# Wangshihu12/Voxel-SLAM

Hardware: AMD Instinct MI355X
Metric: local-BA iterations/sec (200k pts, W=10) (higher is better)
Workload: dtype f64

## Files before the change

include/voxelba.h:

```cpp
#ifndef VOXELBA_H
#define VOXELBA_H

#include <stddef.h>
#include <stdint.h>

#ifdef __cplusplus
extern "C" {
#endif

#define VBA_CLUSTER_LEN 10
#define VBA_POSE_LEN 12
#define VBA_STATE_LEN 25
#define VBA_IMU_PRE_LEN 304
#define VBA_DIM 15
#define VBA_MAX_WIN 16

enum vba_status {
  VBA_OK = 0,
  VBA_ERR_NO_DEVICE = 1,
  VBA_ERR_BAD_ARG = 2,
  VBA_ERR_UNSUPPORTED_WINDOW = 3,
  VBA_ERR_TOO_FEW_VOXELS = 4,
  VBA_ERR_OPT_STATE = 5,
  VBA_ERR_HIP = 6,
  VBA_ERR_CAPACITY = 7,
  VBA_ERR_IO = 8,
  VBA_ERR_UNSUPPORTED = 9,
  VBA_ERR_SINGULAR = 10
};

typedef struct vba_ctx vba_ctx;

typedef struct vba_options {
  int win_size;
  double voxel_size;
  int max_layer;
  int max_points;
  double min_eigen_value;
  double plane_eigen_value_thre[4];
  double min_point[4];
  double imu_coef;
  int thread_num;
  int device;
  void *stream;
  size_t max_voxels;
  size_t max_points_per_scan;
  int lm_spec;
  int force_collective;
  int hessian_workgroups;
  int residual_vpl_from;
  int hessian_compact_tiles;
  size_t max_map_nodes;
  size_t max_fix_points;
  int hba_workers;
  int deterministic;
} vba_options;

void vba_default_options(vba_options *opt);
int vba_create(const vba_options *opt, vba_ctx **out);
void vba_destroy(vba_ctx *ctx);
const char *vba_status_string(int status);
const char *vba_last_error(vba_ctx *ctx);
int vba_synchronize(vba_ctx *ctx);


int vba_factor_clear(vba_ctx *ctx);
int vba_factor_push_voxels(vba_ctx *ctx, int n, const double *clusters, const double *fix, const double *coe,
                           const double *eig_val, const double *eig_vec, const double *pcr_add);
int vba_factor_size(vba_ctx *ctx);
int vba_factor_acc_evaluate2(vba_ctx *ctx, const double *poses, int head, int end, double *Hess, double *JacT,
                             double *residual);
int vba_factor_evaluate_only_residual(vba_ctx *ctx, const double *poses, int head, int end, double *residual);
int vba_factor_read_back(vba_ctx *ctx, double *eig_val, double *eig_vec, double *pcr_add);

int vba_factor_occupied_slots(vba_ctx *ctx, long long *slots);
int vba_factor_occupancy_masks(vba_ctx *ctx, unsigned int *masks);


int vba_lidar_ba_damping_iter(vba_ctx *ctx, double *poses, double *hess, double *resis2, int max_iter, int thd_num,
                              int *is_converge);

int vba_li_ba_damping_iter(vba_ctx *ctx, double *states, double *imus, int gravity, int max_iter, double *hess,
                           double *resis2);

// ... 367 lines not shown
```

voxel-slam_amd/capi.py:

```python
from __future__ import annotations

import ctypes as C
import os
import subprocess

import numpy as np

from .abi import KINDS, PROTOTYPES

_PKG = os.path.dirname(os.path.abspath(__file__))
LIB_PATH = os.environ.get("VBA_LIB") or os.path.join(_PKG, "libvoxelba.so")
_dp = C.POINTER(C.c_double)

OK = 0
ERR_NO_DEVICE, ERR_BAD_ARG, ERR_UNSUPPORTED_WINDOW, ERR_TOO_FEW_VOXELS, ERR_OPT_STATE, ERR_HIP, ERR_CAPACITY, ERR_IO, ERR_UNSUPPORTED, ERR_SINGULAR = range(1, 11)

EXPORTS = list(PROTOTYPES)


class Options(C.Structure):
    _fields_ = [
        ("win_size", C.c_int), ("voxel_size", C.c_double), ("max_layer", C.c_int), ("max_points", C.c_int),
        ("min_eigen_value", C.c_double), ("plane_eigen_value_thre", C.c_double * 4), ("min_point", C.c_double * 4),
        ("imu_coef", C.c_double), ("thread_num", C.c_int), ("device", C.c_int), ("stream", C.c_void_p),
        ("max_voxels", C.c_size_t), ("max_points_per_scan", C.c_size_t),
        ("lm_spec", C.c_int), ("force_collective", C.c_int), ("hessian_workgroups", C.c_int), ("residual_vpl_from", C.c_int), ("hessian_compact_tiles", C.c_int),
        ("max_map_nodes", C.c_size_t), ("max_fix_points", C.c_size_t), ("hba_workers", C.c_int),
        ("deterministic", C.c_int),
    ]


class BtcConfig(C.Structure):
    _fields_ = [
        ("skip_near_num", C.c_int), ("candidate_num", C.c_int), ("rough_dis_threshold", C.c_float),
        ("similarity_threshold", C.c_float), ("icp_threshold", C.c_float), ("normal_threshold", C.c_float),
        ("dis_threshold", C.c_float), ("occupy_len", C.c_int),
    ]


class BtcResult(C.Structure):
    _fields_ = [("loop_id", C.c_int), ("score", C.c_double), ("t", C.c_double * 3), ("R", C.c_double * 9)]


class BtcIcpState(C.Structure):
    _fields_ = [("R", C.c_double * 9), ("t", C.c_double * 3), ("paras", C.c_double * 4), ("is_conv", C.c_int), ("done", C.c_int),
                ("iters", C.c_int), ("pad", C.c_int), ("mat", C.c_double * 6), ("eig", C.c_double * 3)]

    @classmethod
    def start(cls, t, R, paras=(0.2, 0.2, 0.5, 3.0), is_conv=0, done=0, iters=0):
        s = cls()
        s.R[:] = [float(x) for x in np.reshape(R, 9)]; s.t[:] = [float(x) for x in np.reshape(t, 3)]
        s.paras[:] = [float(x) for x in paras]
        s.is_conv, s.done, s.iters = int(is_conv), int(done), int(iters)
        return s


class BtcCandidate(C.Structure):
    _fields_ = [("frame", C.c_int), ("votes", C.c_int), ("match_len", C.c_int), ("max_vote_index", C.c_int),
                ("max_vote", C.c_int), ("score", C.c_double)]
# ... 1454 lines not shown
```

voxel-slam_amd/csrc/vba_ctx.hpp:

```cpp
#pragma once
#include "../../include/voxelba.h"
#include "vba_types.hpp"
#include "vba_common.hpp"
#include "vba_mem.hpp"
#include "vba_stores.hpp"
#include "vba_launch.hpp"

#include <hip/hip_runtime.h>
#include <rccl/rccl.h>
#include <array>
#include <cstdlib>
#include <map>
#include <string>
#include <vector>

using namespace vba;

#define VBA_HIPCHK(err, expr)                                                                    \
  do {                                                                                           \
    hipError_t _e = (expr);                                                                      \
    if (_e != hipSuccess) {                                                                      \
      hipchk_err(err) = std::string(#expr) + ": " + hipGetErrorString(_e);                       \
      return VBA_ERR_HIP;                                                                        \
    }                                                                                            \
// ... 19 lines not shown
}
}
namespace vbh { struct OdomEkf; }
struct CtxSat;

struct vba_ctx {
  vba_options opt;
  int device = 0;
  hipStream_t stream = nullptr;
  bool own_stream = false;
  std::string err;

  FactorView fv{};
  DevMem<double> fv_rows[6];
  DevMem<unsigned int> fv_occ;
  DevMem<int> fv_tiles;
  int nvox = 0;
  int nvox_global = 0;
  int cap = 0;
  DevMem<double> d_poses;
  DevMem<double> d_partial;
  DevMem<double> d_out;
  DevMem<double> d_full;
  DevMem<double> d_scal;
  PinMem<double> h_pin;
  DevMem<char> d_stage;

  vba_allreduce_fn allreduce = nullptr;
  void *allreduce_user = nullptr;
  int rank = 0, n_ranks = 1;
  bool force_collective = false;
  int max_blocks_hess = 256;
  int residual_vpl_from = 45000;
  bool use_h3 = false;
  ncclComm_t comm = nullptr;
  bool own_comm = false;
  bool collective_off = false;
  bool collective() const { return !collective_off && (allreduce || comm) && (n_ranks > 1 || force_collective); }

  bool timing = false;
  std::string timing_only;
  int timing_every = 1; unsigned timing_ctr = 0;
  int lm_spec = LM_SPEC;
  std::vector<std::array<double, 450>> covinv_cache; size_t covinv_next = 0;
  std::map<std::string, std::vector<TimedSpan>> spans;

  DevMem<LmDev> d_lm;
  PinMem<LmDev> h_lm;
  struct { bool pending = false; int dbg = 0; double x[VBA_MAX_WIN_DEV * 12]; } lm_init;
  DevMem<double> d_raw;
  struct { bool active = false; int thd_num = 2; bool have_hess = false; bool pending_update = false; int k4_nb = 0; } lm;
  DevMem<double> d_k4part;
  std::vector<double> trace;

  DevMem<LiDev> d_li;
  DevMem<double> d_imu, d_himu, d_gimu;

  MapStore map;
  GbaStore gba;
  BigStore big;
  DevMem<double> d_refpts;
  DevMem<double> d_lipack;
  DevMem<double> d_liscr;
  DevMem<double> d_hba_all;
  std::vector<vba_ctx *> hba_workers;
  CtxSat *sat = nullptr;
// ... 66 lines not shown
```

voxel-slam_amd/csrc/vba_kernels_factor.hpp:

```cpp
#pragma once
#include <hip/hip_runtime.h>
#include "vba_types.hpp"
#include "vba_common.hpp"
#include "vba_hess_units.hpp"

namespace vba {

__global__ void k_aos_to_soa(FactorView f, int base, int n, const double *__restrict__ clusters, const double *__restrict__ fix,
                             const double *__restrict__ coe, const double *__restrict__ eig_val, const double *__restrict__ eig_vec,
                             const double *__restrict__ pcr_add) {
  const int W = f.W;
  const int per = 10 * W + 10 + 1 + 3 + 9 + 10;
  const long long tot = (long long)n * per;
  for (long long t = (long long)blockIdx.x * blockDim.x + threadIdx.x; t < tot; t += (long long)gridDim.x * blockDim.x) {
    const int a = (int)(t / per);
    int j = (int)(t % per);
    const int v = base + a;
    if (j < 10 * W) {
      const int i = j / 10, fld = j % 10;
      f.cl[((size_t)fld * W + i) * f.vs + v] = clusters[((size_t)a * W + i) * 10 + fld];
      continue;
    }
    j -= 10 * W;
    if (j < 10) { f.fix[(size_t)j * f.vs + v] = fix[(size_t)a * 10 + j]; continue; }
    j -= 10;
    if (j < 1) { f.coe[v] = coe[a]; continue; }
    j -= 1;
    if (j < 3) { f.eigval[(size_t)j * f.vs + v] = eig_val[(size_t)a * 3 + j]; continue; }
    j -= 3;
    if (j < 9) { f.eigvec[(size_t)j * f.vs + v] = eig_vec[(size_t)a * 9 + j]; continue; }
    j -= 9;
    f.pcr[(size_t)j * f.vs + v] = pcr_add[(size_t)a * 10 + j];
  }
}

__global__ void k_soa_to_aos_out(FactorView f, int n, double *__restrict__ eig_val, double *__restrict__ eig_vec, double *__restrict__ pcr_add) {
  const long long tot = (long long)n * 22;
// ... 39 lines not shown

__device__ __forceinline__ int wave_max_to_lane63(int x) {
  auto mx = [](int a, int b) { return a > b ? a : b; };
  x = mx(x, __builtin_amdgcn_update_dpp(x, x, 0xB1, 0xF, 0xF, false));
  x = mx(x, __builtin_amdgcn_update_dpp(x, x, 0x4E, 0xF, 0xF, false));
  x = mx(x, __builtin_amdgcn_update_dpp(x, x, 0x141, 0xF, 0xF, false));
  x = mx(x, __builtin_amdgcn_update_dpp(x, x, 0x140, 0xF, 0xF, false));
  x = mx(x, __builtin_amdgcn_update_dpp(0, x, 0x142, 0xA, 0xF, false));
  x = mx(x, __builtin_amdgcn_update_dpp(0, x, 0x143, 0xC, 0xF, false));
  return x;
}

struct LmDev;
template <int W>
struct LmInit {
  double x[12 * W];
  LmDev *dst;
  int on, dbg;
};
template <int W>
__device__ __forceinline__ void lm_init_store(const LmInit<W> &a, int tid, int nt);
template <int W, int NT>
__device__ __forceinline__ void lm_init_store_lds(const double *sp, LmDev *dst, int dbg, int tid);

template <int W, int TV>
struct ResCfg {
  static constexpr int NT = ((TV * W + 63) / 64) * 64;
  static constexpr int NF = NT / TV;
  static constexpr int KPT = (10 + NF - 1) / NF;
  static_assert(TV <= 64 && (TV & (TV - 1)) == 0 && NT % TV == 0, "the voxel threads are the first TV lanes of wave 0");
  static_assert(W * 12 <= NT, "one thread per pose scalar");
};

template <int W, int TV, bool STAMPS>
__global__ __launch_bounds__((ResCfg<W, TV>::NT)) void k_residual_s(FactorView f, const double *__restrict__ poses, int head, int end,
                                                                  double *__restrict__ partial, const int *__restrict__ gate,
                                                                  long long *__restrict__ stamps, LmInit<W> init) {
  using C = ResCfg<W, TV>;
  __shared__ double T[10][W][TV];
  __shared__ double S[10][TV];
  __shared__ double sp[W * 12];
  const int gate_v = gate ? *gate : 1;
  const int tid = threadIdx.x, vl = tid % TV, fi = tid / TV;
  const int v = head + blockIdx.x * TV + vl;
  const size_t vs = (size_t)f.vs, fs = (size_t)W * vs;
  const int vc = v < end ? v : end - 1;
  const int fic = fi < W ? fi : W - 1;
  long long st0 = 0, st1 = 0, st2 = 0, st3 = 0;
  if (STAMPS) st0 = clock64();
  const unsigned int occm = f.occ[vc];
  const double pose_s = init.on ? init.x[tid < W * 12 ? tid : 0] : poses[tid < W * 12 ? tid : 0];
  double acc[C::KPT];
#pragma unroll
  for (int j = 0; j < C::KPT; j++) { const int k = fi + j * C::NF; acc[j] = f.fix[(size_t)(k < 10 ? k : 9) * vs + vc]; }
  double coe = f.coe[vc];
  unsigned int occv = occm;
  asm volatile("" : "+v"(occv), "+v"(coe), "+v"(acc[0]));
  if (gate_v == 0) return;
  if (tid < W * 12) sp[tid] = pose_s;
  const bool occ = fi < W && v < end && ((occv >> fic) & 1u);
  double c[9], n = 0.0;
#pragma unroll
  for (int k = 0; k < 9; k++) c[k] = occ ? f.cl[(size_t)k * fs + (size_t)fi * vs + v] : 0.0;
  if (occ) n = f.cl[9 * fs + (size_t)fi * vs + v];
  __syncthreads();
  if (init.on && blockIdx.x == 0) lm_init_store_lds<W, C::NT>(sp, init.dst, init.dbg, tid);
  if (occ) {
    const Cl10 w = cluster_transform_exact(c[0], c[1], c[2], c[3], c[4], c[5], c[6], c[7], c[8], n, sp + 12 * fi);
    T[0][fi][vl] = w.p00; T[1][fi][vl] = w.p10; T[2][fi][vl] = w.p20; T[3][fi][vl] = w.p11; T[4][fi][vl] = w.p21; T[5][fi][vl] = w.p22;
    T[6][fi][vl] = w.v0; T[7][fi][vl] = w.v1; T[8][fi][vl] = w.v2;
    T[9][fi][vl] = n;
  } else if (fi < W) {
#pragma unroll
    for (int k = 0; k < 10; k++) T[k][fi][vl] = 0.0;
  }
  __syncthreads();
#pragma unroll
  for (int j = 0; j < C::KPT; j++) {
    const int k = fi + j * C::NF;
    if (k < 10) {
      double a = acc[j];
#pragma unroll
      for (int i = 0; i < W; i++) a += T[k][i][vl];
      S[k][vl] = a;
      if (v < end) f.pcr[(size_t)k * vs + v] = a;
    }
  }
  __syncthreads();
  if (STAMPS) st1 = clock64();
  double r = 0.0;
  if (fi == 0 && v < end) {
    const double Nv = S[9][vl];
    double iN = __builtin_amdgcn_rcp(Nv);
    iN = iN * (2.0 - Nv * iN);
    iN = iN * (2.0 - Nv * iN);
    const double b0 = S[6][vl] * iN, b1 = S[7][vl] * iN, b2 = S[8][vl] * iN;
    double w0, w1, w2, V[9];
    eig3_sym_dev(S[0][vl] * iN - b0 * b0, S[1][vl] * iN - b1 * b0, S[2][vl] * iN - b2 * b0, S[3][vl] * iN - b1 * b1, S[4][vl] * iN - b2 * b1,
                 S[5][vl] * iN - b2 * b2, w0, w1, w2, V);
    if (STAMPS) st2 = clock64();
    f.eigval[0 * vs + v] = w0; f.eigval[1 * vs + v] = w1; f.eigval[2 * vs + v] = w2;
#pragma unroll
    for (int k = 0; k < 9; k++) f.eigvec[(size_t)k * vs + v] = V[k];
    r = coe * w0;
  }
  if (tid < 64) {
    r = wave_sum_to_lane63(r);
    if (tid == 63) partial[blockIdx.x] = r;
    if (STAMPS && tid == 0 && blockIdx.x < 2048) {
      st3 = clock64();
      long long *o = stamps + (size_t)blockIdx.x * 4;
      o[0] = st0; o[1] = st1; o[2] = st2; o[3] = st3;
    }
  }
}

template <int W, bool STAMPS, bool INIT = false>
__global__ __launch_bounds__(64) void k_residual_v(FactorView f, const double *__restrict__ poses, int head, int end,
                                                   double *__restrict__ partial, const int *__restrict__ gate, long long *__restrict__ stamps,
                                                   LmInit<W> init) {
  const int gate_v = gate ? *gate : 1;
  const int lane = threadIdx.x;
  const int v = head + blockIdx.x * 64 + lane;
  const size_t vs = (size_t)f.vs, fs = (size_t)W * vs;
  const int vc = v < end ? v : end - 1;
  long long st0 = 0, st1 = 0, st2 = 0, st3 = 0;
  if (STAMPS) st0 = clock64();
  unsigned int occm = f.occ[vc];
  double acc[10];
#pragma unroll
  for (int k = 0; k < 10; k++) acc[k] = f.fix[(size_t)k * vs + vc];
  double coe = f.coe[vc];
  asm volatile("" : "+v"(occm), "+v"(coe), "+v"(acc[0]));
  if (gate_v == 0) return;
  if (INIT && blockIdx.x == 0) lm_init_store(init, lane, 64);
  if (v >= end) occm = 0;
  double c[W][10];
#pragma unroll
  for (int i = 0; i < W; i++) {
    const bool on = (occm >> i) & 1u;
    if (__ballot(on) != 0ull) {
#pragma unroll
      for (int k = 0; k < 10; k++) c[i][k] = on ? f.cl[(size_t)k * fs + (size_t)i * vs + v] : 0.0;
    } else {
#pragma unroll
      for (int k = 0; k < 10; k++) c[i][k] = 0.0;
    }
// ... 441 lines not shown
```

voxel-slam_amd/csrc/vba_kernels_lm.hpp:

```cpp
#pragma once
#include <hip/hip_runtime.h>
#include "vba_types.hpp"
#include "vba_ldlt.hpp"

namespace vba {


struct LmDev {
  double x[VBA_MAX_WIN_DEV * 12];
  double xt[VBA_MAX_WIN_DEV * 12];
  double u, v, r1, r2, q1, resis_first;
  int is_calc_hess, stop, iter, n_trace, all_accepted, last_accepted, max_trace, run_hess, run_res, pad;
  double trace[5 * 64];
  long long stamps[64];
  int spec_n, spec_i, use_spec, pad2;
  double q1_spec[LM_SPEC];
  double xt_spec[LM_SPEC][VBA_MAX_WIN_DEV * 12];
};

template <int W>
__device__ __forceinline__ void lm_init_store(const LmInit<W> &a, int tid, int nt) {
  constexpr int NW = sizeof(LmDev) / 8, XT = offsetof(LmDev, xt) / 8, U = offsetof(LmDev, u) / 8, V = offsetof(LmDev, v) / 8,
                I = offsetof(LmDev, is_calc_hess) / 8;
  static_assert(sizeof(LmDev) % 8 == 0 && offsetof(LmDev, x) == 0 && offsetof(LmDev, u) == 2 * offsetof(LmDev, xt) && 12 * W <= XT, "x and xt lead the image");
  static_assert(offsetof(LmDev, is_calc_hess) % 8 == 0 && offsetof(LmDev, pad) == offsetof(LmDev, is_calc_hess) + 36, "the ten flags are five words");
  auto two = [](int lo, int hi) { return (unsigned long long)(unsigned int)lo | ((unsigned long long)(unsigned int)hi << 32); };
  unsigned long long *o = reinterpret_cast<unsigned long long *>(a.dst);
  for (int w = tid; w < NW; w += nt) {
    unsigned long long val = 0ull;
    if (w < 2 * XT) { const int k = w < XT ? w : w - XT; if (k < 12 * W) val = (unsigned long long)__double_as_longlong(a.x[k]); }
    else if (w == U) val = (unsigned long long)__double_as_longlong(0.01);
    else if (w == V) val = (unsigned long long)__double_as_longlong(2.0);
    else if (w == I) val = two(1, 0);
    else if (w == I + 2) val = two(1, 0);
    else if (w == I + 3) val = two(64, 1);
    else if (w == I + 4) val = two(1, a.dbg);
    o[w] = val;
  }
}

template <int W, int NT>
__device__ __forceinline__ void lm_init_store_lds(const double *sp, LmDev *dst, int dbg, int tid) {
  constexpr int NW = sizeof(LmDev) / 8, XT = offsetof(LmDev, xt) / 8, U = offsetof(LmDev, u) / 8, V = offsetof(LmDev, v) / 8,
                I = offsetof(LmDev, is_calc_hess) / 8;
  constexpr int NI = (NW + NT - 1) / NT, NP = (2 * XT + NT - 1) / NT;
  static_assert(sizeof(LmDev) % 8 == 0 && offsetof(LmDev, x) == 0 && offsetof(LmDev, u) == 2 * offsetof(LmDev, xt) && 12 * W <= XT, "x and xt lead the image");
  static_assert(offsetof(LmDev, is_calc_hess) % 8 == 0 && offsetof(LmDev, pad) == offsetof(LmDev, is_calc_hess) + 36, "the ten flags are five words");
  auto two = [](int lo, int hi) { return (unsigned long long)(unsigned int)lo | ((unsigned long long)(unsigned int)hi << 32); };
// ... 7 lines not shown
#pragma unroll
  for (int j = 0; j < NI; j++) {
    const int w = tid + j * NT;
    unsigned long long val = 0ull;
    if (j < NP && w < 2 * XT) { const int k = w < XT ? w : w - XT; if (k < 12 * W) val = (unsigned long long)__double_as_longlong(pv[j < NP ? j : 0]); }
    else if (w == U) val = (unsigned long long)__double_as_longlong(0.01);
    else if (w == V) val = (unsigned long long)__double_as_longlong(2.0);
    else if (w == I) val = two(1, 0);
    else if (w == I + 2) val = two(1, 0);
    else if (w == I + 3) val = two(64, 1);
    else if (w == I + 4) val = two(1, dbg);
    if (w < NW) o[w] = val;
  }
}

template <int W>
__global__ __launch_bounds__(256) void k_lm_init(LmInit<W> a) { lm_init_store(a, threadIdx.x, 256); }

__device__ __forceinline__ void so3_exp_dev(const double *w, double *R) {
  const double n = sqrt(w[0] * w[0] + w[1] * w[1] + w[2] * w[2]);
  if (n >= 1e-11) {
    const double a0 = w[0] / n, a1 = w[1] / n, a2 = w[2] / n;
    const double s = sin(n), c1 = 1.0 - cos(n);
    R[0] = 1.0 + c1 * (a0 * a0 - 1.0); R[1] = -s * a2 + c1 * a0 * a1;    R[2] = s * a1 + c1 * a0 * a2;
    R[3] = s * a2 + c1 * a1 * a0;      R[4] = 1.0 + c1 * (a1 * a1 - 1.0); R[5] = -s * a0 + c1 * a1 * a2;
    R[6] = -s * a1 + c1 * a2 * a0;     R[7] = s * a0 + c1 * a2 * a1;     R[8] = 1.0 + c1 * (a2 * a2 - 1.0);
  } else {
    R[0] = 1; R[1] = 0; R[2] = 0; R[3] = 0; R[4] = 1; R[5] = 0; R[6] = 0; R[7] = 0; R[8] = 1;
  }
}



template <int W>
__host__ __device__ __forceinline__ int tl_eidx(int row, int col) {
  using C = HessCfg2<W>;
  const int fr = row / 6;
  if (col / 6 != fr) return -1;
  const int a = row - 6 * fr, b = col - 6 * fr;
  int idx;
  if (b < 3) idx = a * 3 - a * (a - 1) / 2 + (b - a);
  else if (a < 3) idx = 6 + 3 * a + (b - 3);
  else { const int a2 = a - 3, b2 = b - 3; idx = 15 + a2 * 3 - a2 * (a2 - 1) / 2 + (b2 - a2); }
  return C::EB + 21 * fr + idx;
}

template <int W, bool COPY_RAW>
__global__ __launch_bounds__(256) void k_lm_solve_m(LmDev *s, const double *__restrict__ red, double *__restrict__ raw, double *__restrict__ dx_out) {
  const int sb = blockIdx.x;
  using C2 = HessCfg2<W>;
  constexpr int n = 6 * W, NT = 256, NP = ((n + 1 + 15) / 16) * 16, NH = (n + 63) / 64, NU = C2::NU, T16 = C2::NT16;
  using LC = LdltCfg<NP>;
  constexpr int IMG = NP * (NP + 1) / 2, ZERO = (n + 1) * (n + 2) / 2;
  static_assert(IMG <= LC::LTOT && NP >= n + 2, "the image must lie in the L region: ldlt_mfma writes P while the tiles are read");
  __shared__ __attribute__((aligned(16))) double lds[LC::DOUBLES];
  __shared__ double hd[n], gs[n], xs[NP], dxs[n], red8[8];
  __shared__ int ord[n];
  double *Lst = lds, *Tp = Lst + LC::LTOT, *P = Tp + NP * LC::LS, *img = lds;
  const int tid = threadIdx.x, lane = tid & 63, wv = tid >> 6;
  const int use_spec = s->use_spec, stop = s->stop, calc = s->is_calc_hess;
  const double u0 = s->u, v0 = s->v;
  __builtin_amdgcn_sched_barrier(0);
  double dgt[NH], dge[NH], gv[NH];
  auto load_diag = [&](const double *__restrict__ src) {
#pragma unroll
    for (int h = 0; h < NH; h++) {
      const int k = lane + 64 * h, kc = k < n ? k : n - 1, ta = kc >> 4, rt = kc & 15;
      dgt[h] = src[(ta * T16 - ta * (ta - 1) / 2) * 256 + (rt >> 2) * 64 + (rt & 3) * 16 + rt];
      dge[h] = src[tl_eidx<W>(kc, kc)];
      gv[h] = src[C2::GB + kc];
    }
  };
  const int ru = (lane >> 4) + 4 * wv, cu = lane & 15;
  double tv[NU], ev[NU];
  bool eon[NU];
  auto load_bulk = [&](const double *__restrict__ src) {
    int u = 0;
#pragma unroll
    for (int ta = 0; ta < T16; ta++)
#pragma unroll
      for (int tb = ta; tb < T16; tb++, u++) {
        const int row = 16 * ta + ru, col = 16 * tb + cu;
        const int e = (row <= col && col < n) ? tl_eidx<W>(row, col) : -1;
        eon[u] = e >= 0;
        tv[u] = src[u * 256 + tid];
        ev[u] = src[e >= 0 ? e : C2::EB];
      }
  };
  if constexpr (!COPY_RAW) { load_diag(red); load_bulk(red); }
  const double r_v = COPY_RAW ? 0.0 : red[C2::RB];
// ... 69 lines not shown
    }
#pragma unroll
  for (int i = n; i < NP; i++)
    if (tid <= i && (i > n || tid >= n)) img[i * (i + 1) / 2 + tid] = (tid == i) ? 1.0 : 0.0;
  const int iter0 = s->iter, dbg = s->pad;
  if (tid == 0 && calc && sb == 0) { const double r = COPY_RAW ? red[C2::RB] : r_v; s->r1 = r; if (iter0 == 0) s->resis_first = r; }
  long long *stamps = ((dbg & 16) && tid == 0 && sb == 0) ? s->stamps : nullptr;
  if (stamps) stamps[0] = t_begin;
  __syncthreads();
  auto elem = [&](int i, int j) -> double {
    return img[i >= j ? i * (i + 1) / 2 + j : ZERO];
  };
  if (stamps) stamps[1] = clock64();
  const int ncols = (dbg & 128) ? NP : 8 * npan, nsol = ncols < n ? ncols : n;
  ldlt_mfma<NP, NT>(Lst, Tp, P, n, elem, ((dbg & 16) && sb == 0) ? s->stamps : nullptr, LdltDense(), ncols);
  if (stamps) { stamps[3] = clock64(); stamps[6] = (ncols + 7) / 8 < LC::NBLK ? (ncols + 7) / 8 : LC::NBLK; }
  if (tid < n) xs[tid] = tid < nsol ? Lst[LC::lat(n, tid)] : 0.0;
  for (int kb = (nsol + 7) >> 3; 8 * kb < n; kb++)
    for (int e = tid; e < (n - 8 * kb) * LC::LS; e += NT) Lst[LC::lst_off(kb) + e] = 0.0;
  __syncthreads();
  const double x = ldlt_backsub<NP>(Lst, xs, n);
  if (stamps) stamps[4] = clock64();
  if (tid < n) dxs[ord[tid]] = x;
  __syncthreads();
  if (wv == 3) {
    if (lane < W) {
      double E[9];
      so3_exp_dev(dxs + 6 * lane, E);
      const double *R = xr;
      double *Rt = (sb == 0 ? s->xt : s->xt_spec[sb]) + 12 * lane;
#pragma unroll
      for (int r = 0; r < 3; r++)
#pragma unroll
        for (int c = 0; c < 3; c++) Rt[3 * r + c] = R[3 * r] * E[c] + R[3 * r + 1] * E[3 + c] + R[3 * r + 2] * E[6 + c];
#pragma unroll
      for (int k = 0; k < 3; k++) Rt[9 + k] = R[9 + k] + dxs[6 * lane + 3 + k];
    }
    if (lane == 63) red8[3] = 0.0;
  } else {
    double q = tid < n ? dxs[tid] * (u * hd[tid] * dxs[tid] - gs[tid]) : 0.0;
    q = wave_sum_to_lane63(q);
    if (lane == 63) red8[wv] = q;
  }
  __syncthreads();
  if (dx_out && tid < n) dx_out[sb * n + tid] = dxs[tid];
  if (tid == 0) {
    const double q1 = 0.5 * (red8[0] + red8[1] + red8[2] + red8[3]);
    s->q1_spec[sb] = q1;
    if (sb == 0) { s->q1 = q1; s->spec_n = gridDim.x; s->spec_i = 0; }
  }
  if (stamps) stamps[5] = clock64();
}


__device__ int lm_prev_stop(const LmDev *s) { return s->stop; }
__device__ double lm_r1(const LmDev *s) { return s->r1; }
__device__ const double *lm_xt(const LmDev *s) { return s->xt; }

struct LmCand { double q1, p0, p1, p2; };
struct LmUpdIn {
  int stop, ntr, mtr, it, spec_n, spec_i;
  double r1, q1, u0, v0, xt0, xt1, xt2;
  LmCand c;
};
static_assert(VBA_MAX_WIN_DEV * 12 == 192 && LM_SPEC == 4, "three pose words per lane; candidates 1, 2, 3");
__device__ __forceinline__ LmCand lm_cand_load(const LmDev *s, int b, int lane) {
  return {s->q1_spec[b], s->xt_spec[b][lane], s->xt_spec[b][lane + 64], s->xt_spec[b][lane + 128]};
}
__device__ __forceinline__ void lm_update_load(const LmDev *s, int lane, LmUpdIn &in) {
  in.stop = s->stop; in.ntr = s->n_trace; in.mtr = s->max_trace; in.it = s->iter; in.spec_n = s->spec_n; in.spec_i = s->spec_i;
  in.r1 = s->r1; in.q1 = s->q1; in.u0 = s->u; in.v0 = s->v;
  in.xt0 = s->xt[lane]; in.xt1 = s->xt[lane + 64]; in.xt2 = s->xt[lane + 128];
}
__device__ __forceinline__ void lm_pin(LmCand &c) { asm volatile("" : "+v"(c.p0), "+v"(c.p1), "+v"(c.p2)); }
__device__ __forceinline__ void lm_pin(LmUpdIn &in) { asm volatile("" : "+v"(in.xt0), "+v"(in.xt1), "+v"(in.xt2)); }
template <class F>
__device__ __forceinline__ void lm_update_load_all(const LmDev *s, int lane, LmUpdIn &in, F wait) {
  lm_update_load(s, lane, in);
  LmCand c1 = lm_cand_load(s, 1, lane), c2 = lm_cand_load(s, 2, lane), c3 = lm_cand_load(s, 3, lane);
  wait();
  lm_pin(in); lm_pin(c1); lm_pin(c2); lm_pin(c3);
  const int nx = in.spec_i + 1;
  auto pick = [nx](double a1, double a2, double a3) { return nx == 2 ? a2 : nx == 3 ? a3 : a1; };
  in.c = {pick(c1.q1, c2.q1, c3.q1), pick(c1.p0, c2.p0, c3.p0), pick(c1.p1, c2.p1, c3.p1), pick(c1.p2, c2.p2, c3.p2)};
}

// ... 89 lines not shown
```

voxel-slam_amd/csrc/voxelba.hip:

```cpp
#include "vba_ctx.hpp"
#include "vba_kernels_factor.hpp"
#include "vba_kernels_h3.hpp"
#include "vba_kernels_lm.hpp"
#include "vba_kernels_li.hpp"
#include <cstddef>
#include "vba_hostmath.hpp"

#include <hip/hip_runtime.h>
#include <rccl/rccl.h>
#include <dlfcn.h>
#include <cstdio>
#include <cstdlib>
#include <cstring>
#include <string>
#include <vector>
#include <array>
#include <map>
#include <chrono>
#include <algorithm>

using namespace vba;

namespace {

// ... 452 lines not shown
    case VBA_ERR_NO_DEVICE: return "no HIP device (libvoxelba has no CPU path)";
    case VBA_ERR_BAD_ARG: return "bad argument";
    case VBA_ERR_UNSUPPORTED_WINDOW: return "unsupported window size";
    case VBA_ERR_TOO_FEW_VOXELS: return "too few voxels (reference: 'Too Less Voxel' exit)";
    case VBA_ERR_OPT_STATE: return "opt_state out of range (reference: exit)";
    case VBA_ERR_HIP: return "HIP runtime error";
    case VBA_ERR_CAPACITY: return "capacity exceeded";
    case VBA_ERR_IO: return "file missing or malformed";
    case VBA_ERR_UNSUPPORTED: return "not available in this process (RCCL could not be resolved)";
    case VBA_ERR_SINGULAR: return "singular system (a component without a prior, or a non-positive pivot)";
    default: return "unknown";
  }
}

int vba_create(const vba_options *opt, vba_ctx **out) {
  if (!opt || !out) return VBA_ERR_BAD_ARG;
  *out = nullptr;
  if (opt->win_size < 2 || opt->win_size > VBA_MAX_WIN) return VBA_ERR_UNSUPPORTED_WINDOW;
  int ndev = 0;
  if (hipGetDeviceCount(&ndev) != hipSuccess || ndev <= 0) return VBA_ERR_NO_DEVICE;
  vba_ctx *c = new vba_ctx();
  c->opt = *opt;
  if (opt->device >= 0) {
    if (hipSetDevice(opt->device) != hipSuccess) { delete c; return VBA_ERR_NO_DEVICE; }
    c->device = opt->device;
  } else {
    hipGetDevice(&c->device);
  }
  c->lm_spec = opt->lm_spec > 0 ? std::min(opt->lm_spec, (int)LM_SPEC) : (int)LM_SPEC;
  c->force_collective = opt->force_collective != 0;
  c->max_blocks_hess = opt->hessian_workgroups > 0 ? std::min(opt->hessian_workgroups, kMaxBlocksHess) : kMaxBlocksHess;
  if (c->max_blocks_hess < 2) c->max_blocks_hess = 2;
  c->residual_vpl_from = opt->residual_vpl_from > 0 ? opt->residual_vpl_from : 45000;
  c->use_h3 = opt->hessian_compact_tiles != 0 && opt->deterministic == 0;
  if (opt->stream) { c->stream = (hipStream_t)opt->stream; c->own_stream = false; }
  else {
    if (hipStreamCreateWithFlags(&c->stream, hipStreamNonBlocking) != hipSuccess) { delete c; return VBA_ERR_HIP; }
    c->own_stream = true;
  }
  if (int r = ctx_sat_create(c)) { vba_destroy(c); return r; }
  const int W = opt->win_size, nout = nout_of(W);
  c->fv.W = W;
  if (c->d_poses.ensure((size_t)VBA_MAX_WIN * 12) != hipSuccess || c->d_out.ensure((size_t)nout_tl(W) + 64) != hipSuccess ||
      c->d_full.ensure((size_t)nout + 64) != hipSuccess || c->d_scal.ensure(64) != hipSuccess) { vba_destroy(c); return VBA_ERR_HIP; }
  if (ensure_partial(c, (size_t)kMaxBlocksHess * (nout_tl(W) > nout ? nout_tl(W) : nout)) != VBA_OK || ensure_pin(c, kPinCreate + (size_t)nout) != VBA_OK) { vba_destroy(c); return VBA_ERR_HIP; }
  if (c->d_lm.ensure(1) != hipSuccess || c->d_raw.ensure((size_t)nout_tl(W) + 64) != hipSuccess || c->h_lm.ensure(1) != hipSuccess) { vba_destroy(c); return VBA_ERR_HIP; }
  if (opt->max_voxels && factor_reserve(c, (int)opt->max_voxels) != VBA_OK) { vba_destroy(c); return VBA_ERR_HIP; }
  map_init(c->map, c->opt);
  *out = c;
  return VBA_OK;
}

void vba_destroy(vba_ctx *c) {
  if (!c) return;
  hipSetDevice(c->device);
  if (c->stream) hipStreamSynchronize(c->stream);
  if (c->comm && c->own_comm) rccl_api().CommDestroy(c->comm);
  map_free(c->map);
  for (vba_ctx *w : c->hba_workers) vba_destroy(w);
  c->hba_workers.clear();
  ctx_sat_release(c);
  for (auto &kv : c->spans) for (auto &s : kv.second) { hipEventDestroy(s.a); hipEventDestroy(s.b); }
  if (c->own_stream && c->stream) hipStreamDestroy(c->stream);
  delete c;
}

// ... 119 lines not shown
    HIPCHK(c, hipMemcpyAsync(h_count, d_count, sizeof(double), hipMemcpyDeviceToHost, c->stream));
    HIPCHK(c, hipStreamSynchronize(c->stream));
    c->nvox_global = (int)(*h_count + 0.5);
  }
  return VBA_OK;
}

int vba_lm_refresh_eigen(vba_ctx *c) {
  if (!c->lm.active) return VBA_ERR_BAD_ARG;
  if (c->nvox <= 0) return VBA_OK;
  if ((size_t)residual_nb(c, c->nvox) > c->d_partial.n) { c->set_error("partial buffer too small"); return VBA_ERR_CAPACITY; }
  TimedSpan s1{};
  span_begin(c, "residual", s1);
  const bool fuse_init = !c->collective();
  if (!fuse_init) { const int st = lm_init_flush(c); if (st) return st; }
  const int st = launch_residual(c, lm_ptrs(c).x, nullptr, 0, c->nvox, nullptr, fuse_init);
  if (st) return st;
  span_end(c, "residual", s1);
  HIPCHK(c, hipGetLastError());
  return VBA_OK;
}

int vba_timing_launch_hessian(vba_ctx *c) {
  if (!c->lm.active || c->nvox <= 0) return VBA_ERR_BAD_ARG;
  int nb = 0;
  int st = lm_init_flush(c);
  if (st) return st;
  st = launch_hessian(c, lm_ptrs(c).x, nullptr, 0, c->nvox, &nb, PassCargo{});
  if (st) return st;
  HIPCHK(c, hipGetLastError());
  return VBA_OK;
}

int vba_lm_iterate(vba_ctx *c, int *accepted, int *stop) {
  if (!c->lm.active) return VBA_ERR_BAD_ARG;
  const int W = c->opt.win_size, nout = nout_of(W), V = c->nvox;
  if (c->nvox_global < c->lm.thd_num) { c->lm_init.pending = false; return VBA_ERR_TOO_FEW_VOXELS; }
  const LmPtrs p = lm_ptrs(c);
  const int copy_raw = c->collective() ? 1 : 0;
  int st = VBA_OK;
  static const bool no_fuse = diag_env("VBA_NO_FUSED_UPDATE") != nullptr;
  if (copy_raw) { st = lm_init_flush(c); if (st) return st; }
  if (needs_hessian_pass(c)) {
    st = hessian_pass(c, p.x, p.run_hess, 0, V, c->lm.pending_update ? cargo_pending_update(c) : cargo_call_init());
    c->lm.pending_update = false;
  }
  if (st) return st;
  TimedSpan sp{};
  span_begin(c, "solve", sp);
  st = for_window<2, 16>(W, [&](auto wc) {
    constexpr int WW = decltype(wc)::value;
    if (copy_raw) hipLaunchKernelGGL((k_lm_solve_m<WW, true>), dim3(c->lm_spec), dim3(256), 0, c->stream, c->d_lm, c->d_out, c->d_raw, nullptr);
    else hipLaunchKernelGGL((k_lm_solve_m<WW, false>), dim3(c->lm_spec), dim3(256), 0, c->stream, c->d_lm, c->d_out, c->d_raw, nullptr);
    return VBA_OK;
  });
  if (st) return st;
  span_end(c, "solve", sp);
  if (copy_raw) {
    st = sharded_trial_step(c, p, V, [&](const double *r) { hipLaunchKernelGGL(k_lm_update, dim3(1), dim3(64), 0, c->stream, c->d_lm, r, 0, W); });
    if (st) return st;
  } else {
    const int nb = residual_nb(c, V);
    if ((size_t)nb > c->d_k4part.n) {
      if (c->d_k4part) HIPCHK(c, hipStreamSynchronize(c->stream));
      HIPCHK(c, c->d_k4part.ensure(nb > 65536 ? 2 * (size_t)nb : 65536));
    }
    const bool fuse = !no_fuse && !(accepted || stop);
    TimedSpan s1{};
    span_begin(c, "residual", s1);
    st = launch_residual(c, p.xt, p.run_res, 0, V, c->d_k4part);
    if (st) return st;
    span_end(c, "residual", s1);
    if (fuse) { c->lm.pending_update = true; c->lm.k4_nb = nb; }
    else hipLaunchKernelGGL(k_lm_update, dim3(1), dim3(64), 0, c->stream, c->d_lm, c->d_k4part, nb, W);
  }
  HIPCHK(c, hipGetLastError());
  if (accepted || stop) {
    HIPCHK(c, hipMemcpyAsync(c->h_lm, c->d_lm, sizeof(LmDev), hipMemcpyDeviceToHost, c->stream));
    HIPCHK(c, hipStreamSynchronize(c->stream));
    if (accepted) *accepted = c->h_lm->last_accepted;
    if (stop) *stop = c->h_lm->stop;
  }
  return VBA_OK;
}

int vba_lm_end(vba_ctx *c, double *poses, double *hess, double *resis2) {
  if (!c->lm.active) return VBA_ERR_BAD_ARG;
  const int W = c->opt.win_size, n = 6 * W;
  const bool want = poses || hess || resis2;
  if (!want && !c->lm.pending_update) { c->lm_init.pending = false; c->lm.active = false; return VBA_OK; }
  int st = lm_init_flush(c);
  if (st) return st;
  if (!want) {
    hipLaunchKernelGGL(k_lm_update, dim3(1), dim3(64), 0, c->stream, c->d_lm, c->d_k4part, c->lm.k4_nb, W);
    c->lm.pending_update = false;
    c->lm.active = false;
    return VBA_OK;
  }
  double *h_hess = nullptr;
  if (hess) {
    st = ensure_pin(c, kPinCreate + (size_t)n * n);
    if (st) return st;
    h_hess = c->h_pin + kPinStage;
  }
  const double *src = c->collective() ? c->d_raw : c->d_out;
  const int upd = c->lm.pending_update ? 1 : 0;
  st = for_window<2, 16>(W, [&](auto wc) {
    hipLaunchKernelGGL(k_lm_finish<decltype(wc)::value>, dim3(hess ? 17 : 1), dim3(256), 0, c->stream, c->d_lm, c->d_k4part, upd ? c->lm.k4_nb : 0, upd, c->h_lm, src, h_hess);
    return VBA_OK;
  });
  if (st) return st;
  c->lm.pending_update = false;
  HIPCHK(c, hipGetLastError());
  HIPCHK(c, hipStreamSynchronize(c->stream));
  const LmDev *h = c->h_lm;
  if (poses) std::memcpy(poses, h->x, (size_t)W * 12 * sizeof(double));
  if (hess) std::memcpy(hess, h_hess, (size_t)n * n * sizeof(double));
  if (resis2) { resis2[0] = h->resis_first; resis2[1] = h->r2; }
  c->trace.assign(h->trace, h->trace + 5 * h->n_trace);
  solve_cycles_dump("k_lm_solve_m", h, 8);
  c->lm.active = false;
  return VBA_OK;
}

int vba_lidar_ba_damping_iter(vba_ctx *c, double *poses, double *hess, double *resis2, int max_iter, int thd_num, int *is_converge) {
  int st = vba_lm_begin(c, poses, thd_num);
  if (st) return st;
  for (int i = 0; i < max_iter; i++) {
    st = vba_lm_iterate(c, nullptr, nullptr);
    if (st) { c->lm.active = false; return st; }
  }
  st = vba_lm_end(c, poses, hess, resis2);
  if (is_converge) *is_converge = c->h_lm->all_accepted;
  return st;
}

int vba_last_lm_trace(vba_ctx *c, double *rows, int max_rows) {
  int n = (int)(c->trace.size() / 5);
  if (n > max_rows) n = max_rows;
  if (rows) std::memcpy(rows, c->trace.data(), (size_t)n * 5 * sizeof(double));
  return n;
}

extern "C++" {
template <int W>
struct LiSolveCfg {
  static constexpr int NMAX = 15 * W + 3, NP = ((NMAX + 1 + 15) / 16) * 16;
  static constexpr bool GL = W > 10;
  static constexpr size_t l_doubles = (size_t)LdltCfg<NP>::LTOT > (size_t)NMAX * (NMAX + 1) / 2 ? (size_t)LdltCfg<NP>::LTOT : (size_t)NMAX * (NMAX + 1) / 2;
  static constexpr size_t lds = ((GL ? (size_t)LdltCfg<NP>::DOUBLES - LdltCfg<NP>::LTOT : (size_t)LdltCfg<NP>::DOUBLES) + 4 * NMAX + NP + 32) * 8 + (size_t)NMAX * 4 + 64;
  static_assert(GL || l_doubles == (size_t)LdltCfg<NP>::LTOT, "the staged triangle must fit the region of L");
};
template <int W, int NT = (W > 10 ? 1024 : 512)>
static int launch_li_solve(vba_ctx *c, int copy_raw, int n, int gauge, int grav) {
// ... 576 lines not shown
```

Baseline: 23880.

## Fuse LM solve and trial residual into one kernel with intra-grid handoff

Merges the LM solve kernel and the trial-pose residual kernel into a single launch. Residual workgroups prefetch cluster data, then spin on a sequence flag until solve block 0 publishes trial poses with agent-scope atomic stores. This removes one kernel launch and the gap between the two kernels per iteration. In exchange it relies on all workgroups being co-resident (guarded by a CU-count check), and a timeout fault path marks the step rejected.

Result: faster. 24930 (median of 6 runs) (+4.4%).

```diff
diff --git a/include/voxelba.h b/include/voxelba.h
--- a/include/voxelba.h
+++ b/include/voxelba.h
@@ -50,6 +50,7 @@
   int hessian_workgroups;
   int residual_vpl_from;
   int hessian_compact_tiles;
+  int lm_trial_launches;
   size_t max_map_nodes;
   size_t max_fix_points;
   int hba_workers;
diff --git a/voxel-slam_amd/capi.py b/voxel-slam_amd/capi.py
--- a/voxel-slam_amd/capi.py
+++ b/voxel-slam_amd/capi.py
@@ -25,6 +25,7 @@
         ("imu_coef", C.c_double), ("thread_num", C.c_int), ("device", C.c_int), ("stream", C.c_void_p),
         ("max_voxels", C.c_size_t), ("max_points_per_scan", C.c_size_t),
         ("lm_spec", C.c_int), ("force_collective", C.c_int), ("hessian_workgroups", C.c_int), ("residual_vpl_from", C.c_int), ("hessian_compact_tiles", C.c_int),
+        ("lm_trial_launches", C.c_int),
         ("max_map_nodes", C.c_size_t), ("max_fix_points", C.c_size_t), ("hba_workers", C.c_int),
         ("deterministic", C.c_int),
     ]
diff --git a/voxel-slam_amd/csrc/vba_ctx.hpp b/voxel-slam_amd/csrc/vba_ctx.hpp
--- a/voxel-slam_amd/csrc/vba_ctx.hpp
+++ b/voxel-slam_amd/csrc/vba_ctx.hpp
@@ -75,6 +75,7 @@
   bool force_collective = false;
   int max_blocks_hess = 256;
   int residual_vpl_from = 45000;
+  bool lm_trial_fused = true;
   bool use_h3 = false;
   ncclComm_t comm = nullptr;
   bool own_comm = false;
diff --git a/voxel-slam_amd/csrc/vba_kernels_factor.hpp b/voxel-slam_amd/csrc/vba_kernels_factor.hpp
--- a/voxel-slam_amd/csrc/vba_kernels_factor.hpp
+++ b/voxel-slam_amd/csrc/vba_kernels_factor.hpp
@@ -3,6 +3,7 @@
 #include "vba_types.hpp"
 #include "vba_common.hpp"
 #include "vba_hess_units.hpp"
+#include <type_traits>
 
 namespace vba {
 
@@ -108,39 +109,63 @@
   static_assert(W * 12 <= NT, "one thread per pose scalar");
 };
 
-template <int W, int TV, bool STAMPS>
-__global__ __launch_bounds__((ResCfg<W, TV>::NT)) void k_residual_s(FactorView f, const double *__restrict__ poses, int head, int end,
-                                                                  double *__restrict__ partial, const int *__restrict__ gate,
-                                                                  long long *__restrict__ stamps, LmInit<W> init) {
+template <int W, int TV>
+struct ResLds {
+  alignas(16) double T[10][W][TV];
+  alignas(16) double S[10][TV];
+  alignas(16) double sp[W * 12];
+};
+struct NoRider {};
+
+template <int W, int TV, bool STAMPS, class RIDER>
+__device__ __forceinline__ void residual_s_body(ResLds<W, TV> &L, const int bid, const FactorView &f, const double *__restrict__ poses, int head, int end,
+                                                double *__restrict__ partial, const int *__restrict__ gate, long long *__restrict__ stamps,
+                                                const LmInit<W> &init, RIDER rider) {
   using C = ResCfg<W, TV>;
-  __shared__ double T[10][W][TV];
-  __shared__ double S[10][TV];
-  __shared__ double sp[W * 12];
-  const int gate_v = gate ? *gate : 1;
+  constexpr bool RIDES = !std::is_same<RIDER, NoRider>::value;
+  auto &T = L.T; auto &S = L.S; auto &sp = L.sp;
+  int gate_v = 1;
+  if constexpr (!RIDES) gate_v = gate ? *gate : 1;
   const int tid = threadIdx.x, vl = tid % TV, fi = tid / TV;
-  const int v = head + blockIdx.x * TV + vl;
+  const int v = head + bid * TV + vl;
   const size_t vs = (size_t)f.vs, fs = (size_t)W * vs;
   const int vc = v < end ? v : end - 1;
   const int fic = fi < W ? fi : W - 1;
   long long st0 = 0, st1 = 0, st2 = 0, st3 = 0;
   if (STAMPS) st0 = clock64();
   const unsigned int occm = f.occ[vc];
-  const double pose_s = init.on ? init.x[tid < W * 12 ? tid : 0] : poses[tid < W * 12 ? tid : 0];
+  double pose_s;
+  if constexpr (RIDES) pose_s = rider.request(W * 12, tid);
+  else pose_s = init.on ? init.x[tid < W * 12 ? tid : 0] : poses[tid < W * 12 ? tid : 0];
   double acc[C::KPT];
 #pragma unroll
   for (int j = 0; j < C::KPT; j++) { const int k = fi + j * C::NF; acc[j] = f.fix[(size_t)(k < 10 ? k : 9) * vs + vc]; }
   double coe = f.coe[vc];
   unsigned int occv = occm;
   asm volatile("" : "+v"(occv), "+v"(coe), "+v"(acc[0]));
+  if constexpr (RIDES) gate_v = rider.run();
   if (gate_v == 0) return;
-  if (tid < W * 12) sp[tid] = pose_s;
+  if constexpr (!RIDES) { if (tid < W * 12) sp[tid] = pose_s; }
   const bool occ = fi < W && v < end && ((occv >> fic) & 1u);
   double c[9], n = 0.0;
 #pragma unroll
   for (int k = 0; k < 9; k++) c[k] = occ ? f.cl[(size_t)k * fs + (size_t)fi * vs + v] : 0.0;
   if (occ) n = f.cl[9 * fs + (size_t)fi * vs + v];
+  if constexpr (RIDES) {
+    if (!rider.have_xt()) {
+#pragma unroll
+      for (int k = 0; k < 9; k++) asm volatile("" : "+v"(c[k]));
+      asm volatile("" : "+v"(n));
+      if (!rider.wait(tid)) {
+        if (tid == 0) { partial[bid] = __builtin_nan(""); rider.fault(); }
+        return;
+      }
+      pose_s = rider.xt(W * 12, tid);
+    }
+    if (tid < W * 12) sp[tid] = pose_s;
+  }
   __syncthreads();
-  if (init.on && blockIdx.x == 0) lm_init_store_lds<W, C::NT>(sp, init.dst, init.dbg, tid);
+  if constexpr (!RIDES) { if (init.on && bid == 0) lm_init_store_lds<W, C::NT>(sp, init.dst, init.dbg, tid); }
   if (occ) {
     const Cl10 w = cluster_transform_exact(c[0], c[1], c[2], c[3], c[4], c[5], c[6], c[7], c[8], n, sp + 12 * fi);
     T[0][fi][vl] = w.p00; T[1][fi][vl] = w.p10; T[2][fi][vl] = w.p20; T[3][fi][vl] = w.p11; T[4][fi][vl] = w.p21; T[5][fi][vl] = w.p22;
@@ -182,13 +207,21 @@
   }
   if (tid < 64) {
     r = wave_sum_to_lane63(r);
-    if (tid == 63) partial[blockIdx.x] = r;
-    if (STAMPS && tid == 0 && blockIdx.x < 2048) {
+    if (tid == 63) partial[bid] = r;
+    if (STAMPS && tid == 0 && bid < 2048) {
       st3 = clock64();
-      long long *o = stamps + (size_t)blockIdx.x * 4;
+      long long *o = stamps + (size_t)bid * 4;
       o[0] = st0; o[1] = st1; o[2] = st2; o[3] = st3;
     }
   }
+}
+
+template <int W, int TV, bool STAMPS>
+__global__ __launch_bounds__((ResCfg<W, TV>::NT)) void k_residual_s(FactorView f, const double *__restrict__ poses, int head, int end,
+                                                                  double *__restrict__ partial, const int *__restrict__ gate,
+                                                                  long long *__restrict__ stamps, LmInit<W> init) {
+  __shared__ ResLds<W, TV> L;
+  residual_s_body<W, TV, STAMPS, NoRider>(L, blockIdx.x, f, poses, head, end, partial, gate, stamps, init, NoRider{});
 }
 
 template <int W, bool STAMPS, bool INIT = false>
diff --git a/voxel-slam_amd/csrc/vba_kernels_lm.hpp b/voxel-slam_amd/csrc/vba_kernels_lm.hpp
--- a/voxel-slam_amd/csrc/vba_kernels_lm.hpp
+++ b/voxel-slam_amd/csrc/vba_kernels_lm.hpp
@@ -2,6 +2,7 @@
 #include <hip/hip_runtime.h>
 #include "vba_types.hpp"
 #include "vba_ldlt.hpp"
+#include "vba_kernels_factor.hpp"
 
 namespace vba {
 
@@ -13,7 +14,8 @@
   int is_calc_hess, stop, iter, n_trace, all_accepted, last_accepted, max_trace, run_hess, run_res, pad;
   double trace[5 * 64];
   long long stamps[64];
-  int spec_n, spec_i, use_spec, pad2;
+  int spec_n, spec_i, use_spec, xt_seq;
+  int trial_fault, pad3;
   double q1_spec[LM_SPEC];
   double xt_spec[LM_SPEC][VBA_MAX_WIN_DEV * 12];
 };
@@ -87,6 +89,12 @@
 
 
 
+template <bool PUB>
+__device__ __forceinline__ void lm_xt_store(double *p, double v) {
+  if constexpr (PUB) __hip_atomic_store(p, v, __ATOMIC_RELAXED, __HIP_MEMORY_SCOPE_AGENT);
+  else *p = v;
+}
+
 template <int W>
 __host__ __device__ __forceinline__ int tl_eidx(int row, int col) {
   using C = HessCfg2<W>;
@@ -100,17 +108,28 @@
   return C::EB + 21 * fr + idx;
 }
 
-template <int W, bool COPY_RAW>
-__global__ __launch_bounds__(256) void k_lm_solve_m(LmDev *s, const double *__restrict__ red, double *__restrict__ raw, double *__restrict__ dx_out) {
-  const int sb = blockIdx.x;
+template <int W>
+struct LmSolveLds {
+  static constexpr int n = 6 * W, NP = ((n + 1 + 15) / 16) * 16;
+  alignas(16) double lds[LdltCfg<NP>::DOUBLES];
+  alignas(16) double hd[n];
+  alignas(16) double gs[n];
+  alignas(16) double xs[NP];
+  alignas(16) double dxs[n];
+  alignas(16) double red8[8];
+  alignas(16) int ord[n];
+};
+
+template <int W, bool COPY_RAW, bool PUBLISH>
+__device__ __forceinline__ void lm_solve_body(LmSolveLds<W> &L, const int sb, const int nspec, LmDev *s, const double *__restrict__ red, double *__restrict__ raw,
+                                              double *__restrict__ dx_out) {
   using C2 = HessCfg2<W>;
   constexpr int n = 6 * W, NT = 256, NP = ((n + 1 + 15) / 16) * 16, NH = (n + 63) / 64, NU = C2::NU, T16 = C2::NT16;
   using LC = LdltCfg<NP>;
   constexpr int IMG = NP * (NP + 1) / 2, ZERO = (n + 1) * (n + 2) / 2;
   static_assert(IMG <= LC::LTOT && NP >= n + 2, "the image must lie in the L region: ldlt_mfma writes P while the tiles are read");
-  __shared__ __attribute__((aligned(16))) double lds[LC::DOUBLES];
-  __shared__ double hd[n], gs[n], xs[NP], dxs[n], red8[8];
-  __shared__ int ord[n];
+  double *lds = L.lds, *hd = L.hd, *gs = L.gs, *xs = L.xs, *dxs = L.dxs, *red8 = L.red8;
+  int *ord = L.ord;
   double *Lst = lds, *Tp = Lst + LC::LTOT, *P = Tp + NP * LC::LS, *img = lds;
   const int tid = threadIdx.x, lane = tid & 63, wv = tid >> 6;
   const int use_spec = s->use_spec, stop = s->stop, calc = s->is_calc_hess;
@@ -246,9 +265,15 @@
 #pragma unroll
       for (int r = 0; r < 3; r++)
 #pragma unroll
-        for (int c = 0; c < 3; c++) Rt[3 * r + c] = R[3 * r] * E[c] + R[3 * r + 1] * E[3 + c] + R[3 * r + 2] * E[6 + c];
-#pragma unroll
-      for (int k = 0; k < 3; k++) Rt[9 + k] = R[9 + k] + dxs[6 * lane + 3 + k];
+        for (int c = 0; c < 3; c++) lm_xt_store<PUBLISH>(Rt + 3 * r + c, R[3 * r] * E[c] + R[3 * r + 1] * E[3 + c] + R[3 * r + 2] * E[6 + c]);
+#pragma unroll
+      for (int k = 0; k < 3; k++) lm_xt_store<PUBLISH>(Rt + 9 + k, R[9 + k] + dxs[6 * lane + 3 + k]);
+    }
+    if constexpr (PUBLISH) {
+      if (sb == 0) {
+        asm volatile("s_waitcnt vmcnt(0)" ::: "memory");
+        if (lane == 0) __hip_atomic_store(&s->xt_seq, iter0 + 1, __ATOMIC_RELAXED, __HIP_MEMORY_SCOPE_AGENT);
+      }
     }
     if (lane == 63) red8[3] = 0.0;
   } else {
@@ -261,11 +286,72 @@
   if (tid == 0) {
     const double q1 = 0.5 * (red8[0] + red8[1] + red8[2] + red8[3]);
     s->q1_spec[sb] = q1;
-    if (sb == 0) { s->q1 = q1; s->spec_n = gridDim.x; s->spec_i = 0; }
+    if (sb == 0) { s->q1 = q1; s->spec_n = nspec; s->spec_i = 0; }
   }
   if (stamps) stamps[5] = clock64();
 }
 
+template <int W, bool COPY_RAW>
+__global__ __launch_bounds__(256) void k_lm_solve_m(LmDev *s, const double *__restrict__ red, double *__restrict__ raw, double *__restrict__ dx_out) {
+  __shared__ LmSolveLds<W> L;
+  lm_solve_body<W, COPY_RAW, false>(L, blockIdx.x, gridDim.x, s, red, raw, dx_out);
+}
+
+
+constexpr long long kLmTrialWaitTicks = 2000000;
+
+struct LmTrialRider {
+  LmDev *s;
+  int *ok_lds;
+  int run_res, stop, use_spec, iter;
+  __device__ __forceinline__ double request(int npose, int tid) {
+    run_res = s->run_res; stop = s->stop; use_spec = s->use_spec; iter = s->iter;
+    return __hip_atomic_load(&s->xt[tid < npose ? tid : 0], __ATOMIC_RELAXED, __HIP_MEMORY_SCOPE_AGENT);
+  }
+  __device__ __forceinline__ int run() const { return (run_res != 0 && stop == 0) ? 1 : 0; }
+  __device__ __forceinline__ bool have_xt() const { return use_spec != 0; }
+  __device__ __forceinline__ bool wait(int tid) const {
+    if (tid == 0) {
+      const int want = iter + 1;
+      int ok = 1;
+      const long long t0 = wall_clock64();
+      while (__hip_atomic_load(&s->xt_seq, __ATOMIC_RELAXED, __HIP_MEMORY_SCOPE_AGENT) != want) {
+        __builtin_amdgcn_s_sleep(8);
+        if (wall_clock64() - t0 > kLmTrialWaitTicks) { ok = 0; break; }
+      }
+      *ok_lds = ok;
+    }
+    __syncthreads();
+    return *ok_lds != 0;
+  }
+  __device__ __forceinline__ double xt(int npose, int tid) const {
+    return __hip_atomic_load(&s->xt[tid < npose ? tid : 0], __ATOMIC_RELAXED, __HIP_MEMORY_SCOPE_AGENT);
+  }
+  __device__ __forceinline__ void fault() const { __hip_atomic_store(&s->trial_fault, 1, __ATOMIC_RELAXED, __HIP_MEMORY_SCOPE_AGENT); }
+};
+
+template <int W, int TV>
+struct LmTrialCfg {
+  static constexpr int RNT = ResCfg<W, TV>::NT, BS = RNT > 256 ? RNT : 256;
+  union Lds { LmSolveLds<W> solve; ResLds<W, TV> res; };
+};
+
+template <int W, bool COPY_RAW = false, int TV = 32>
+__global__ __launch_bounds__((LmTrialCfg<W, TV>::BS)) void k_lm_trial(LmDev *s, const double *__restrict__ red, double *__restrict__ raw, int nspec, FactorView f,
+                                                                    int head, int end, double *__restrict__ partial) {
+  using TC = LmTrialCfg<W, TV>;
+  __shared__ typename TC::Lds L;
+  __shared__ int wait_ok;
+  if ((int)blockIdx.x < nspec) {
+    if (threadIdx.x >= 256) return;
+    lm_solve_body<W, COPY_RAW, true>(L.solve, blockIdx.x, nspec, s, red, raw, nullptr);
+  } else {
+    if (threadIdx.x >= TC::RNT) return;
+    LmInit<W> none;
+    none.on = 0;
+    residual_s_body<W, TV, false, LmTrialRider>(L.res, (int)blockIdx.x - nspec, f, nullptr, head, end, partial, nullptr, nullptr, none, LmTrialRider{s, &wait_ok});
+  }
+}
 
 __device__ int lm_prev_stop(const LmDev *s) { return s->stop; }
 __device__ double lm_r1(const LmDev *s) { return s->r1; }
diff --git a/voxel-slam_amd/csrc/voxelba.hip b/voxel-slam_amd/csrc/voxelba.hip
--- a/voxel-slam_amd/csrc/voxelba.hip
+++ b/voxel-slam_amd/csrc/voxelba.hip
@@ -508,6 +508,7 @@
   c->max_blocks_hess = opt->hessian_workgroups > 0 ? std::min(opt->hessian_workgroups, kMaxBlocksHess) : kMaxBlocksHess;
   if (c->max_blocks_hess < 2) c->max_blocks_hess = 2;
   c->residual_vpl_from = opt->residual_vpl_from > 0 ? opt->residual_vpl_from : 45000;
+  c->lm_trial_fused = opt->lm_trial_launches != 2;
   c->use_h3 = opt->hessian_compact_tiles != 0 && opt->deterministic == 0;
   if (opt->stream) { c->stream = (hipStream_t)opt->stream; c->own_stream = false; }
   else {
@@ -693,6 +694,30 @@
   return VBA_OK;
 }
 
+extern "C++" {
+template <int W>
+struct LmTrialFits { static constexpr bool value = sizeof(typename LmTrialCfg<W, VBA_K4_TV>::Lds) + 16 <= 160 * 1024 / 3 && LmTrialCfg<W, VBA_K4_TV>::BS <= 320; };
+static bool lm_trial_fused(vba_ctx *c, int V, int nb, int copy_raw) {
+  if (!c->lm_trial_fused || copy_raw || V <= 0 || residual_vpl(c, V) || c->lm_init.dbg != 0 || k4_stamps_buffer(c)) return false;
+  bool fits = false;
+  for_window<2, 16>(c->opt.win_size, [&](auto wc) { fits = LmTrialFits<decltype(wc)::value>::value; return VBA_OK; });
+  if (!fits) return false;
+  static std::atomic<int> cus[kMaxDevices] = {};
+  const bool known = c->device >= 0 && c->device < kMaxDevices;
+  int n = known ? cus[c->device].load(std::memory_order_relaxed) : 0;
+  if (n == 0) {
+    if (hipDeviceGetAttribute(&n, hipDeviceAttributeMultiprocessorCount, c->device) != hipSuccess || n <= 0) return false;
+    if (known) cus[c->device].store(n, std::memory_order_relaxed);
+  }
+  return c->lm_spec + nb <= 3 * n;
+}
+static bool lm_trial_fault_seen(vba_ctx *c) {
+  if (c->h_lm->trial_fault == 0) return false;
+  c->set_error("k_lm_trial: a residual workgroup gave up waiting for the solve's trial poses (the step was rejected)");
+  return true;
+}
+}
+
 int vba_lm_iterate(vba_ctx *c, int *accepted, int *stop) {
   if (!c->lm.active) return VBA_ERR_BAD_ARG;
   const int W = c->opt.win_size, nout = nout_of(W), V = c->nvox;
@@ -707,11 +732,22 @@
     c->lm.pending_update = false;
   }
   if (st) return st;
+  const int nb = residual_nb(c, V);
+  if (!copy_raw && (size_t)nb > c->d_k4part.n) {
+    if (c->d_k4part) HIPCHK(c, hipStreamSynchronize(c->stream));
+    HIPCHK(c, c->d_k4part.ensure(nb > 65536 ? 2 * (size_t)nb : 65536));
+  }
+  const bool fused_trial = lm_trial_fused(c, V, nb, copy_raw);
   TimedSpan sp{};
   span_begin(c, "solve", sp);
   st = for_window<2, 16>(W, [&](auto wc) {
     constexpr int WW = decltype(wc)::value;
-    if (copy_raw) hipLaunchKernelGGL((k_lm_solve_m<WW, true>), dim3(c->lm_spec), dim3(256), 0, c->stream, c->d_lm, c->d_out, c->d_raw, nullptr);
+    if (fused_trial) {
+      if constexpr (LmTrialFits<WW>::value)
+        hipLaunchKernelGGL((k_lm_trial<WW, false, VBA_K4_TV>), dim3(c->lm_spec + nb), dim3(LmTrialCfg<WW, VBA_K4_TV>::BS), 0, c->stream, c->d_lm, c->d_out, c->d_raw, c->lm_spec,
+                           c->fv, 0, V, c->d_k4part.p);
+    }
+    else if (copy_raw) hipLaunchKernelGGL((k_lm_solve_m<WW, true>), dim3(c->lm_spec), dim3(256), 0, c->stream, c->d_lm, c->d_out, c->d_raw, nullptr);
     else hipLaunchKernelGGL((k_lm_solve_m<WW, false>), dim3(c->lm_spec), dim3(256), 0, c->stream, c->d_lm, c->d_out, c->d_raw, nullptr);
     return VBA_OK;
   });
@@ -721,17 +757,14 @@
     st = sharded_trial_step(c, p, V, [&](const double *r) { hipLaunchKernelGGL(k_lm_update, dim3(1), dim3(64), 0, c->stream, c->d_lm, r, 0, W); });
     if (st) return st;
   } else {
-    const int nb = residual_nb(c, V);
-    if ((size_t)nb > c->d_k4part.n) {
-      if (c->d_k4part) HIPCHK(c, hipStreamSynchronize(c->stream));
-      HIPCHK(c, c->d_k4part.ensure(nb > 65536 ? 2 * (size_t)nb : 65536));
+    const bool fuse = !no_fuse && !(accepted || stop);
+    if (!fused_trial) {
+      TimedSpan s1{};
+      span_begin(c, "residual", s1);
+      st = launch_residual(c, p.xt, p.run_res, 0, V, c->d_k4part);
+      if (st) return st;
+      span_end(c, "residual", s1);
     }
-    const bool fuse = !no_fuse && !(accepted || stop);
-    TimedSpan s1{};
-    span_begin(c, "residual", s1);
-    st = launch_residual(c, p.xt, p.run_res, 0, V, c->d_k4part);
-    if (st) return st;
-    span_end(c, "residual", s1);
     if (fuse) { c->lm.pending_update = true; c->lm.k4_nb = nb; }
     else hipLaunchKernelGGL(k_lm_update, dim3(1), dim3(64), 0, c->stream, c->d_lm, c->d_k4part, nb, W);
   }
@@ -741,6 +774,7 @@
     HIPCHK(c, hipStreamSynchronize(c->stream));
     if (accepted) *accepted = c->h_lm->last_accepted;
     if (stop) *stop = c->h_lm->stop;
+    if (lm_trial_fault_seen(c)) return VBA_ERR_HIP;
   }
   return VBA_OK;
 }
@@ -781,6 +815,7 @@
   c->trace.assign(h->trace, h->trace + 5 * h->n_trace);
   solve_cycles_dump("k_lm_solve_m", h, 8);
   c->lm.active = false;
+  if (lm_trial_fault_seen(c)) return VBA_ERR_HIP;
   return VBA_OK;
 }
 
```
